# TheCacophonyProject/audio-training

Measured on AMD Instinct MI355X. Metric: clips/sec training (3s@48kHz, wr_resnet) at 1/2/4/8 GPU; mel pipeline GB/s, higher is better.
Workload: dtype bf16

## Files before the change

audio-training_amd/acfe/_lib.py:

```python
from __future__ import annotations

import ctypes as C
import os
from pathlib import Path

LIB_PATH = Path(os.environ.get("ACFE_LIB") or Path(__file__).resolve().parent / "libacfe.so")

P = C.c_void_p
I32 = C.c_int
I64 = C.c_int64
F32 = C.c_float
F64 = C.c_double

SIGNATURES: dict[str, list] = {
    "acfe_version": [],
    "acfe_last_error": [],
    "acfe_crc32c": [P, C.c_size_t, C.c_uint32],
    "acfe_tfr_open": [C.c_char_p, I32, P],
    "acfe_tfr_next": [P, I32, P, P],
    "acfe_tfr_close": [P],
    "acfe_example_audio": [P, C.c_uint64, C.c_char_p, P, I64, P, I32, P],
    "acfe_mel_filterbank": [I32, I32, F64, F64, I32, F64, P],
    "acfe_plan_create": [I32, I32, I32, I32, F64, F64, F64, P, P],
    "acfe_plan_destroy": [P],
# ... 27 lines not shown
    "acfe_conv2d_wgrad_bnbwd_rows": [I32] * 5,
    "acfe_conv2d_wgrad_bnbwd": [P, I32, I32, I32, I32, P, P, I32, P, P, I32, P, P, F32, C.c_uint64, P, P, F32, P, P,
                                P],
    "acfe_conv2d_dropout_keep_supported": [I32] * 6,
    "acfe_conv2d_fwd_dropout_keep": [P, I32, I32, I32, I32, P, I32, I32, I32, P, P, P, F32, C.c_uint64, P, P],
    "acfe_conv2d_fwd_bn_keep": [P, I32, I32, I32, I32, P, I32, I32, I32, P, P, P, F32, C.c_uint64, P, P, I32, P, P,
                                I32, P],
    "acfe_conv2d_wgrad_bnbwd_keep": [P, I32, I32, I32, I32, P, P, I32, P, P, I32, P, F32, C.c_uint64, P, P, P, F32,
                                     P, P, P],
    "acfe_stem_blocks": [I32, I32, I32],
    "acfe_stem_fold_weights": [P, I32, I32, I32, I32, P, P],
    "acfe_stem_fwd": [P, I32, I32, I32, I32, I32, I32, I32, I32, P, P, P, I32, P, P],
    "acfe_stem_dgrad": [P, I32, I32, I32, I32, I32, I32, I32, I32, P, P, I32, P],
    "acfe_stem_wgrad": [P, I32, P, I32, I32, I32, I32, I32, I32, I32, I32, I32, P, F32, P, P],
    "acfe_stem_bwd_bn": [P, P, P, I32, I32, I32, I32, I32, I32, I32, P, P, P, P, I32, P, I32, P, F32, P, P, P],
    "acfe_reduce_blocks": [I64],
    "acfe_bn_stats": [P, I64, I32, I32, P, P],
    "acfe_bn_finalize": [P, I32, I32, I32, F64, P, P, F32, F32, P, P, I32, P, P, P, P, P],
    "acfe_bn_apply": [P, I32, I64, I32, P, P, I32, P, I32, P],
    "acfe_bn_bwd_reduce": [P, I32, P, I32, I64, I32, P, P, P, P, I32, P, P],
    "acfe_bn_bwd_finalize": [P, I32, I32, F64, P, P, P, P, P, P, P],
    "acfe_bn_bwd_finalize_ex": [P, I32, I32, F64, P, P, P, P, P, P, I32, P],
    "acfe_bn_bwd_apply": [P, I32, P, I32, I64, I32, P, P, I32, P, P, P, I32, P],
    "acfe_bn_bwd_apply_dropout": [P, I32, P, I32, I64, I32, P, P, I32, P, F32, C.c_uint64, P, I32, P],
    "acfe_bn_bwd_apply_ex": [P, I32, P, I32, I64, I32, P, P, I32, P, P, F32, C.c_uint64, P, I32, P, P],
    "acfe_conv2d_pool_supported": [I32, I32, I32, I32, I32, I32, I32, I32],
    "acfe_conv2d_fwd_pool": [P, I32, I32, I32, I32, P, I32, I32, I32, P, P, P, F32, C.c_uint64, P, I32, P],
    "acfe_conv2d_dgrad_unpool": [P, P, I32, I32, I32, I32, P, I32, I32, I32, P, I32, P],
    "acfe_conv2d_wgrad_unpool": [P, I32, I32, I32, I32, P, P, I32, I32, I32, P, F32, I32, P, P],
    "acfe_bn_bwd_apply_pool": [P, I32, P, I32, I32, I32, I32, I32, P, P, I32, P, P, I32, P, I32, P, P],
# ... 17 lines not shown
    "acfe_channel_sum": [P, I64, I32, I32, P, P, F32, P],
    "acfe_add": [P, P, I64, I32, P, I32, P],
    "acfe_add_stats": [P, P, I64, I32, I32, P, I32, P, P],
    "acfe_relu_bwd_sum": [P, P, I64, I32, P, I32, P, P],
    "acfe_channel_sum_finalize": [P, I32, I32, F32, P, P],
    "acfe_relu_bwd": [P, P, I64, P, I32, P],
    "acfe_dropout": [P, I64, F32, C.c_uint64, P, I32, P],
    "acfe_cast": [P, I32, I64, P, I32, P],
    "acfe_sigmoid": [P, I64, P, P],
    "acfe_maxpool2d": [P, I32, I32, I32, I32, I32, I32, P, I32, P],
    "acfe_maxpool2d_bwd": [P, P, I32, I32, I32, I32, I32, I32, P, I32, P],
    "acfe_maxpool2d_fused": [P, I32, I32, I32, I32, I32, I32, P, P, F32, C.c_uint64, P, I32, P],
    "acfe_bn_maxpool2d_fused": [P, I32, I32, I32, I32, P, P, I32, I32, I32, P, P, P, I32, P],
    "acfe_maxpool2d_bwd_argmax": [P, P, I32, I32, I32, I32, I32, I32, F32, C.c_uint64, P, I32, P],
    "acfe_maxpool2d_bwd_argmax_bn": [P, P, I32, I32, I32, I32, I32, I32, P, I32, P, P, P, P, P, I32, P, P],
    "acfe_avgpool2d": [P, I32, I32, I32, I32, I32, P, I32, P],
    "acfe_avgpool2d_bwd": [P, I32, I32, I32, I32, I32, P, I32, P],
    "acfe_axis_pool": [P, I32, I64, I32, I32, F32, I32, P, P],
    "acfe_axis_pool_bwd": [P, I32, P, I64, I32, I32, F32, I32, P, P],
    "acfe_dense_fwd": [P, P, P, I32, I32, I32, P, P],
    "acfe_dense_bwd": [P, P, P, I32, I32, I32, P, P, P, P],
    "acfe_loss": [P, P, I32, I32, I32, F32, P, P, P, P],
    "acfe_adam_step": [P, P, P, P, I64, F32, F32, F32, F32, F32, P],
}
_RESTYPES = {"acfe_last_error": C.c_char_p, "acfe_conv2d_wgrad_workspace": I64, "acfe_conv2d_dgrad_workspace": I64, "acfe_crc32c": C.c_uint32,
             "acfe_c1bn_workspace": I64}

PAD_END, PAD_CENTER_CONSTANT, PAD_CENTER_REFLECT = 0, 1, 2
LAYOUT_BTM, LAYOUT_BMT = 0, 1
DTYPE_F32, DTYPE_BF16 = 0, 1
# ... 40 lines not shown
```

audio-training_amd/acfe/ops.py:

```python
from __future__ import annotations

import itertools
import os

import torch

from ._lib import call, lib
from ._torch import dtype_code, ptr, stream

F32, F64 = torch.float32, torch.float64

FUSE = os.environ.get("ACFE_FUSE", "1") != "0"
UNPOOL = os.environ.get("ACFE_UNPOOL", "1") != "0"
PROLOGUE = os.environ.get("ACFE_BN_PROLOGUE", "1") != "0"
PRO_POOL = os.environ.get("ACFE_BN_PROLOGUE_POOL", "1") != "0"
PRO_C1 = os.environ.get("ACFE_BN_PROLOGUE_C1", "0") != "0"
PRO_1W = os.environ.get("ACFE_BN_PROLOGUE_1W", "1") != "0"
FUSE_BN_REDUCE = FUSE and os.environ.get("ACFE_BN_REDUCE_FUSE", "1") != "0"
STEM_BN_FUSE = os.environ.get("ACFE_STEM_BN_FUSE", "1") != "0"
FUSE_BN_BWD = FUSE and os.environ.get("ACFE_BN_BWD_FUSE", "1") != "0"
KEEP_BITS = os.environ.get("ACFE_KEEP_BITS", "1") != "0"
FUSE_SUB = FUSE and os.environ.get("ACFE_SUB_FUSE", "1") != "0"


def same_padding(n: int, k: int, s: int) -> tuple[int, int]:
    out = -(-n // s)
    total = max((out - 1) * s + k - n, 0)
    return out, total // 2


def valid_out(n: int, k: int, s: int) -> int:
    return (n - k) // s + 1


# ... 371 lines not shown
        ctx.save_for_backward(x, w, weff, y, amax, *saved)
        ctx.conf, ctx.gb = conf, (gamma, beta)
        ctx.mark_non_differentiable(pst)
        return yp, pst

    @staticmethod
    def backward(ctx, g, _gs):
        x, w, weff, y, amax, *saved = ctx.saved_tensors
        pt, pl, out_dtype, kh, kw, relu, eps, momentum, want_stats = ctx.conf
        N, H, W, K = y.shape
        _, R, S, rep = w.shape
        dev = y.device
        s = stream()
        scale, shift, mean, invstd = saved
        g = g.contiguous()
        gu = _empty(y.shape, g.dtype, dev)
        rows = N * H * W
        nrows = lib.acfe_reduce_blocks(rows)
        part = _empty((nrows * 2 * K,), F64, dev)
        call("acfe_maxpool2d_bwd_argmax_bn", ptr(amax), ptr(g), N, H, W, K, kh, kw, ptr(gu), dtype_code(g.dtype),
             ptr(y), ptr(scale), ptr(shift), ptr(mean), ptr(invstd), int(relu), ptr(part), s)
        coef, dgamma, dbeta = _bn_bwd_coef(part, nrows, K, rows, saved, True, ctx.gb, dev)
        nb = lib.acfe_stem_blocks(N, H, W)
        dx = _empty(x.shape, x.dtype, dev)
        dw = _empty(w.shape, F32, dev)
        ws = _empty((nb * K * R * S,), F64, dev)
        bp = _empty((nb, 2, K), F64, dev)
        call("acfe_stem_bwd_bn", ptr(gu), ptr(y), ptr(x), N, H, W, R, S, pt, pl, ptr(weff), ptr(scale), ptr(shift),
             ptr(coef), int(relu), ptr(dx), rep, ptr(dw), 0.0, ptr(bp), ptr(ws), s)
        db = None
        if ctx.needs_input_grad[2]:
            db = _empty((K,), F32, dev)
            call("acfe_channel_sum_finalize", ptr(bp), nb, K, 0.0, ptr(db), s)
        return (dx if ctx.needs_input_grad[0] else None), dw, db, dgamma, dbeta, None, None, None


def stem_bn_pool_ok(x, w, b, out_dtype, kh, kw) -> bool:
    K, R, S, _ = w.shape
    return (FUSE and FUSE_BN_REDUCE and STEM_BN_FUSE and torch.is_grad_enabled() and b is not None
            and x.dtype == torch.bfloat16 and out_dtype == torch.bfloat16 and x.dim() == 3 and x.is_contiguous()
            and K == 16 and R == S and R in (3, 5) and (kh, kw) in ((1, 2), (2, 2), (3, 3)))


def stem_bn_max_pool(x, w, b, out_dtype, gamma, beta, mmean, mvar, kh, kw, relu=False, eps=1e-3, momentum=0.99,
# ... 1094 lines not shown
```

audio-training_amd/csrc/conv.hip:

```cpp
#include "conv_common.h"

#if !defined(ACFE_ABLATE) && (defined(ACFE_FB_NOXFORM) || defined(ACFE_FB_NOSUM) || defined(ACFE_FB_NOSTORE) || \
                              defined(ACFE_FB_MID))
#error "ACFE_FB_* ablation switches belong to `make ablate` builds only"
#endif

using namespace acfe;



__device__ __attribute__((aligned(64))) uint4 g_zero_page[4];


template <typename T> struct TT;
template <> struct TT<uint16_t> { static constexpr int GR = 8, BK = 64; };
template <> struct TT<float> { static constexpr int GR = 4, BK = 32; };

__device__ __forceinline__ void mma(f4& acc, const uint4& a, const uint4& b, uint16_t) {
  acc = __builtin_amdgcn_mfma_f32_16x16x32_bf16(__builtin_bit_cast(bf8, a), __builtin_bit_cast(bf8, b), acc,
                                                0, 0, 0);
}
__device__ __forceinline__ void mma(f4& acc, const uint4& a, const uint4& b, float) {
  acc = __builtin_amdgcn_mfma_f32_16x16x4f32(__uint_as_float(a.x), __uint_as_float(b.x), acc, 0, 0, 0);
  acc = __builtin_amdgcn_mfma_f32_16x16x4f32(__uint_as_float(a.y), __uint_as_float(b.y), acc, 0, 0, 0);
// ... 4852 lines not shown
  }
#pragma unroll
  for (int r = 0; r < 4; ++r) {
    red[wid][q * 4 + r][l16] = d0[r];
    red[wid][q * 4 + r][16 + l16] = d1[r];
  }
  __syncthreads();
  for (int i = tid; i < STEM_K * NT; i += 256) {
    const int k = i / NT, t = i - k * NT;
    part[(long long)blockIdx.x * STEM_K * NT + i] =
        ((double)red[0][k][t] + (double)red[1][k][t]) + ((double)red[2][k][t] + (double)red[3][k][t]);
  }
}


template <int R, int S>
__global__ void __launch_bounds__(256) __attribute__((amdgpu_waves_per_eu(3)))
k_stem_bwd_bn(const uint16_t* __restrict__ g, const uint16_t* __restrict__ xb, const uint16_t* __restrict__ xin,
              int N, int H, int W, int pt, int pl, const float* __restrict__ weff, const float* __restrict__ scale,
              const float* __restrict__ shift, const float* __restrict__ coef, int relu, uint16_t* __restrict__ dxin,
              double* __restrict__ wpart, double* __restrict__ bpart, int tiles_h, int tiles_w) {
  constexpr int XH = STEM_TH + R - 1, XW = STEM_TW + S - 1, NT = R * S, NKT = (NT + 1) / 2;
  constexpr int GSZ = XH * XW * STEM_K;
  static_assert(GSZ * 2 >= 4 * STEM_K * 32 * 4, "the wgrad reduction aliases the dY image");
  __shared__ __attribute__((aligned(16))) uint16_t gs[GSZ];
  __shared__ uint16_t xs[XH * XW];
  __shared__ double bred[4][STEM_K];
  __shared__ __attribute__((aligned(16))) float bnc[5][STEM_K];
  const int tid = threadIdx.x, lane = tid & 63, l16 = lane & 15, q = lane >> 4, wid = tid >> 6;
  if (tid < 5 * STEM_K) {
    const int a = tid / STEM_K, k = tid - a * STEM_K;
    bnc[a][k] = a == 0 ? scale[k] : (a == 1 ? shift[k] : coef[(a - 2) * STEM_K + k]);
  }
  uint4 wa[NKT];
  int goff[NKT];
#pragma unroll
  for (int kt = 0; kt < NKT; ++kt) {
    const int t = 2 * kt + (q >> 1), r = t / S, s = t % S;
    float v[8];
#pragma unroll
    for (int j = 0; j < 8; ++j) v[j] = t < NT ? weff[t * STEM_K + (q & 1) * 8 + j] : 0.f;
    wa[kt] = uint4{stem_pack2(v[0], v[1]), stem_pack2(v[2], v[3]), stem_pack2(v[4], v[5]), stem_pack2(v[6], v[7])};
    goff[kt] = t < NT ? ((R - 1 - r) * XW + (S - 1 - s)) * STEM_K + (q & 1) * 8 : -1;
  }
  const int grp = lane >> 4, qq = (lane & 15) >> 2, pp = lane & 3;
  int tof0, tof1;
  {
    const int t0 = l16, t1 = 16 + l16;
    tof0 = t0 < NT ? (t0 / S) * XW + (t0 % S) : -1;
    tof1 = t1 < NT ? (t1 / S) * XW + (t1 % S) : -1;
  }
  const int c8 = (tid & 1) * 8;
  double s1[8];
#pragma unroll
  for (int j = 0; j < 8; ++j) s1[j] = 0.0;
  f4 d0 = f4{0.f, 0.f, 0.f, 0.f}, d1 = d0;
  const uint4 z4 = {0u, 0u, 0u, 0u};
  const long long ntiles = (long long)N * tiles_h * tiles_w;
  for (long long tt = blockIdx.x; tt < ntiles; tt += gridDim.x) {
    const int tw = (int)(tt % tiles_w), th = (int)((tt / tiles_w) % tiles_h);
    const int n = (int)(tt / ((long long)tiles_w * tiles_h));
    const int h0 = th * STEM_TH, w0 = tw * STEM_TW;
    const int gh0 = h0 - (R - 1 - pt), gw0 = w0 - (S - 1 - pl);
    __syncthreads();
    for (int i = tid; i < XH * XW * 2; i += 256) {
      const int pos = i >> 1;
      const int yy = pos / XW, xx = pos - yy * XW;
      const int h = gh0 + yy, w = gw0 + xx;
      u32x4 v = {0u, 0u, 0u, 0u};
      if ((unsigned)h < (unsigned)H && (unsigned)w < (unsigned)W) {
        const long long e = (((long long)n * H + h) * W + w) * STEM_K + c8;
        const u32x4 gv = *reinterpret_cast<const u32x4*>(g + e);
        const u32x4 xv = *reinterpret_cast<const u32x4*>(xb + e);
        float o[8];
#pragma unroll
        for (int j = 0; j < 8; ++j) {
          const unsigned gw = gv[j >> 1], xw = xv[j >> 1];
          const float gf = __uint_as_float((j & 1) ? (gw & 0xffff0000u) : (gw << 16));
          const float xf = __uint_as_float((j & 1) ? (xw & 0xffff0000u) : (xw << 16));
          const float gj = (relu && !(xf * bnc[0][c8 + j] + bnc[1][c8 + j] > 0.f)) ? 0.f : gf;
          o[j] = __builtin_fmaf(bnc[2][c8 + j], gj, __builtin_fmaf(bnc[3][c8 + j], xf, bnc[4][c8 + j]));
        }
        v = u32x4{stem_pack2(o[0], o[1]), stem_pack2(o[2], o[3]), stem_pack2(o[4], o[5]), stem_pack2(o[6], o[7])};
        if ((unsigned)(yy - (R - 1 - pt)) < (unsigned)STEM_TH && (unsigned)(xx - (S - 1 - pl)) < (unsigned)STEM_TW) {
#pragma unroll
          for (int j = 0; j < 8; ++j) {
            const unsigned vw = v[j >> 1];
            s1[j] += (double)__uint_as_float((j & 1) ? (vw & 0xffff0000u) : (vw << 16));
          }
        }
      }
      *reinterpret_cast<u32x4*>(gs + (long long)i * 8) = v;
    }
    for (int i = tid; i < XH * XW; i += 256) {
      const int yy = i / XW, xx = i - yy * XW;
      const int h = h0 - pt + yy, w = w0 - pl + xx;
      xs[i] = ((unsigned)h < (unsigned)H && (unsigned)w < (unsigned)W) ? xin[((long long)n * H + h) * W + w] : 0;
    }
    __syncthreads();
#pragma unroll 2
    for (int blk = 0; blk < 16; ++blk) {
      const int ry = wid * 4 + (blk >> 2), cx = (blk & 3) * 16 + l16;
      const uint16_t* base = gs + (ry * XW + cx) * STEM_K;
      f4 acc = f4{0.f, 0.f, 0.f, 0.f};
#pragma unroll
      for (int kt = 0; kt < NKT; ++kt) {
        const uint4 b = goff[kt] >= 0 ? *reinterpret_cast<const uint4*>(base + goff[kt]) : z4;
        acc = __builtin_amdgcn_mfma_f32_16x16x32_bf16(__builtin_bit_cast(bf8, wa[kt]), __builtin_bit_cast(bf8, b), acc,
                                                      0, 0, 0);
      }
      const int h = h0 + ry, w = w0 + cx;
      if (q == 0 && h < H && w < W) dxin[((long long)n * H + h) * W + w] = f2bf(acc[0]);
    }
    for (int c = 0; c < 8; ++c) {
// ... 5 lines not shown
          (stem_lp)(reinterpret_cast<const __bf16*>(gw + (16 + 4 * grp + qq) * STEM_K + 4 * pp)));
      const bf8 a = bf8{lo[0], lo[1], lo[2], lo[3], hi[0], hi[1], hi[2], hi[3]};
      const uint16_t* src = xs + ry * XW + cx0;
      unsigned b0[8], b1[8];
#pragma unroll
      for (int j = 0; j < 8; ++j) {
        const int px = j < 4 ? 4 * q + j : 16 + 4 * q + (j - 4);
        b0[j] = tof0 >= 0 ? src[px + tof0] : 0u;
        b1[j] = tof1 >= 0 ? src[px + tof1] : 0u;
      }
      const uint4 B0 = uint4{b0[0] | (b0[1] << 16), b0[2] | (b0[3] << 16), b0[4] | (b0[5] << 16), b0[6] | (b0[7] << 16)};
      const uint4 B1 = uint4{b1[0] | (b1[1] << 16), b1[2] | (b1[3] << 16), b1[4] | (b1[5] << 16), b1[6] | (b1[7] << 16)};
      d0 = __builtin_amdgcn_mfma_f32_16x16x32_bf16(a, __builtin_bit_cast(bf8, B0), d0, 0, 0, 0);
      d1 = __builtin_amdgcn_mfma_f32_16x16x32_bf16(a, __builtin_bit_cast(bf8, B1), d1, 0, 0, 0);
    }
  }
#pragma unroll
  for (int j = 0; j < 8; ++j) {
#pragma unroll
    for (int o = 2; o < 64; o <<= 1) s1[j] += __shfl_xor(s1[j], o, 64);
  }
  __syncthreads();
  float(*red)[STEM_K][32] = reinterpret_cast<float(*)[STEM_K][32]>(gs);
#pragma unroll
  for (int r = 0; r < 4; ++r) {
    red[wid][q * 4 + r][l16] = d0[r];
    red[wid][q * 4 + r][16 + l16] = d1[r];
  }
  if (lane < 2) {
#pragma unroll
// ... 103 lines not shown
      hipLaunchKernelGGL((k_stem_wgrad_mfma<3, 3>), dim3(grid), dim3(256), 0, strm(stream), (const uint16_t*)x,
                         (const uint16_t*)dy, N, H, W, pad_top, pad_left, workspace, th, tw);
  } else if (x_dtype == ACFE_DTYPE_BF16 && dy_dtype == ACFE_DTYPE_BF16) SW(uint16_t, uint16_t);
  else if (x_dtype == ACFE_DTYPE_BF16) SW(uint16_t, float);
  else if (dy_dtype == ACFE_DTYPE_BF16) SW(float, uint16_t);
  else SW(float, float);
#undef SW
  int rc = launch_rc("acfe_stem_wgrad");
  if (rc) return rc;
  const int n = STEM_K * R * S;
  if (rep > 256) return ACFE_E_INVAL;
  hipLaunchKernelGGL(k_stem_wgrad_reduce, dim3(n), dim3(256), 0, strm(stream), workspace, grid, n, rep, beta, dw);
  return launch_rc("acfe_stem_wgrad(reduce)");
}

ACFE_API int acfe_stem_bwd_bn(const void* g, const void* xb, const void* xin, int N, int H, int W, int R, int S,
                              int pad_top, int pad_left, const float* weff, const float* scale, const float* shift,
                              const float* coef, int relu, void* dxin, int rep, float* dw, float beta,
                              double* bias_part, double* workspace, void* stream) {
  if (!g || !xb || !xin || !weff || !scale || !shift || !coef || !dw || !bias_part || !workspace || N <= 0 ||
      H <= 0 || W <= 0 || R != S || (R != 5 && R != 3) || rep <= 0 || rep > 256 || ((uintptr_t)g & 15) ||
      ((uintptr_t)xb & 15))
    return ACFE_E_INVAL;
  const int th = (H + STEM_TH - 1) / STEM_TH, tw = (W + STEM_TW - 1) / STEM_TW;
  const int nb = acfe_stem_blocks(N, H, W), grid = stem_bwd_grid(N, H, W);
  if (grid < nb) {
    const hipError_t e =
        hipMemsetAsync(bias_part + (size_t)grid * 2 * STEM_K, 0, sizeof(double) * 2 * STEM_K * (nb - grid), strm(stream));
    if (e != hipSuccess) return hip_rc(e, "acfe_stem_bwd_bn");
  }
  uint16_t* dxo = (uint16_t*)dxin;
  if (!dxo) return ACFE_E_INVAL;
#define SB(RR)                                                                                                \
  hipLaunchKernelGGL((k_stem_bwd_bn<RR, RR>), dim3(grid), dim3(256), 0, strm(stream), (const uint16_t*)g,        \
                     (const uint16_t*)xb, (const uint16_t*)xin, N, H, W, pad_top, pad_left, weff, scale, shift, coef, \
                     relu, dxo, workspace, bias_part, th, tw)
  if (R == 5) SB(5); else SB(3);
#undef SB
  int rc = launch_rc("acfe_stem_bwd_bn");
  if (rc) return rc;
  const int n = STEM_K * R * S;
  hipLaunchKernelGGL(k_stem_wgrad_reduce, dim3(n), dim3(256), 0, strm(stream), workspace, grid, n, rep, beta, dw);
  return launch_rc("acfe_stem_bwd_bn(reduce)");
}
```

audio-training_amd/csrc/nn.hip:

```cpp
#include "common.h"

using namespace acfe;

template <typename T> __device__ __forceinline__ float ld(const T* p, long long i);
template <> __device__ __forceinline__ float ld<uint16_t>(const uint16_t* p, long long i) { return bf2f(p[i]); }
template <> __device__ __forceinline__ float ld<float>(const float* p, long long i) { return p[i]; }
template <typename T> __device__ __forceinline__ void st(T* p, long long i, float v);
template <> __device__ __forceinline__ void st<uint16_t>(uint16_t* p, long long i, float v) { p[i] = f2bf(v); }
template <> __device__ __forceinline__ void st<float>(float* p, long long i, float v) { p[i] = v; }

#define DISPATCH1(dt, T, ...)                                   \
  do {                                                          \
    if ((dt) == ACFE_DTYPE_BF16) { typedef uint16_t T; __VA_ARGS__; } \
    else { typedef float T; __VA_ARGS__; }                      \
  } while (0)

static int grid_for(long long n, int per = 256, int cap = 8192) {
  long long g = (n + per - 1) / per;
  if (g < 1) g = 1;
  return (int)(g < cap ? g : cap);
}

static int red_blocks(long long rows) {
  long long b = (rows + 255) / 256;
// ... 1053 lines not shown
        st8(dx + (((size_t)n * H + p * KH + a) * W + q * KW + b) * C + cv * 8, o);
      }
    const float z[8] = {0, 0, 0, 0, 0, 0, 0, 0};
    if (q == Q - 1)
      for (int a = 0; a < KH; ++a)
        for (int w = Q * KW; w < W; ++w) st8(dx + (((size_t)n * H + p * KH + a) * W + w) * C + cv * 8, z);
    if (p == P - 1)
      for (int h = P * KH; h < H; ++h) {
        for (int w = q * KW; w < q * KW + KW; ++w) st8(dx + (((size_t)n * H + h) * W + w) * C + cv * 8, z);
        if (q == Q - 1)
          for (int w = Q * KW; w < W; ++w) st8(dx + (((size_t)n * H + h) * W + w) * C + cv * 8, z);
      }
  }
}

template <typename T, int KH, int KW>
__global__ void __launch_bounds__(256) k_maxpool_bwd8i_bn(const uint8_t* __restrict__ amax, const T* __restrict__ dy,
                                                          int N, int H, int W, int C, int P, int Q,
                                                          T* __restrict__ dx, const T* __restrict__ x,
                                                          const float* __restrict__ scale,
                                                          const float* __restrict__ shift,
                                                          const float* __restrict__ mean,
                                                          const float* __restrict__ invstd, int relu,
                                                          double* __restrict__ part) {
  extern __shared__ double red[];
  for (int i = threadIdx.x; i < 2 * C; i += 256) red[i] = 0.0;
  __syncthreads();
  constexpr int JU = 2;
  const int CV = C >> 3, lcv = __builtin_ctz(CV), RV = Q * CV;
  const int cv = threadIdx.x & (CV - 1);
  float sc[8], sh[8], mu[8], is[8], a[8], b[8];
// ... 33 lines not shown
#pragma unroll
        for (int k = 0; k < 4; ++k) am[k] = (pk[u].x >> (8 * k)) & 0xff, am[4 + k] = (pk[u].y >> (8 * k)) & 0xff;
#pragma unroll
        for (int aa = 0; aa < KH; ++aa)
#pragma unroll
          for (int bb = 0; bb < KW; ++bb) {
            const float* xw = xv[u][aa * KW + bb];
            float o[8];
#pragma unroll
            for (int k = 0; k < 8; ++k) {
              o[k] = am[k] == aa * KW + bb ? g[u][k] : 0.f;
              const float gk = (relu && !(xw[k] * sc[k] + sh[k] > 0.f)) ? 0.f : o[k];
              a[k] += gk;
              b[k] += gk * ((xw[k] - mu[k]) * is[k]);
            }
            st8(dx + (fin + ((size_t)aa * W + q * KW + bb) * CV + cv) * 8, o);
          }
        if (q == Q - 1)
          for (int aa = 0; aa < KH; ++aa)
            for (int w = Q * KW; w < W; ++w) st8(dx + (fin + ((size_t)aa * W + w) * CV + cv) * 8, z);
        if (p == P - 1)
          for (int h = P * KH; h < H; ++h) {
            const size_t hr = ((size_t)n * H + h) * W;
            for (int w = q * KW; w < q * KW + KW; ++w) st8(dx + ((hr + w) * CV + cv) * 8, z);
            if (q == Q - 1)
              for (int w = Q * KW; w < W; ++w) st8(dx + ((hr + w) * CV + cv) * 8, z);
          }
      }
    }
    if (++cnt == 16) {
#pragma unroll
      for (int j = 0; j < 8; ++j) da[j] += a[j], db[j] += b[j], a[j] = b[j] = 0.f;
// ... 76 lines not shown
      kw <= 0 || H < kh || W < kw || !stats8_ok(C))
    return ACFE_E_INVAL;
  const int P = H / kh, Q = W / kw;
  if (!vec_ok((long long)N * H * W * C, C, dy, dx, x) || ((uintptr_t)argmax & 7) || (long long)N * P >= (1ll << 31))
    return ACFE_E_INVAL;
  const int grid = red_blocks((long long)N * H * W);
#define MPBB(A, B)                                                                                             \
  if (kh == A && kw == B) {                                                                                    \
    DISPATCH1(dtype, T, hipLaunchKernelGGL((k_maxpool_bwd8i_bn<T, A, B>), dim3(grid), dim3(256),               \
                                           2 * C * sizeof(double), strm(stream), argmax, (const T*)dy, N, H, W, C, \
                                           P, Q, (T*)dx, (const T*)x, scale, shift, mean, invstd, relu, part));   \
    return launch_rc("acfe_maxpool2d_bwd_argmax_bn");                                                          \
  }
  MAXPOOL_SHAPES(MPBB)
#undef MPBB
  return ACFE_E_INVAL;
}

template <typename T>
__global__ void __launch_bounds__(256) k_add8s(const T* __restrict__ a, const T* __restrict__ b, unsigned nvec,
                                               int C, int relu, T* __restrict__ z, double* __restrict__ part) {
  extern __shared__ double red[];
  for (int i = threadIdx.x; i < 2 * C; i += 256) red[i] = 0.0;
  __syncthreads();
  const int CV = C >> 3;
  double sa[8], sb[8];
#pragma unroll
  for (int j = 0; j < 8; ++j) sa[j] = sb[j] = 0.0;
  const unsigned v0 = blockIdx.x * 256 + threadIdx.x;
  for (unsigned v = v0; v < nvec; v += gridDim.x * 256) {
// ... 452 lines not shown
```

include/acfe.h:

```cpp
#ifndef ACFE_H
#define ACFE_H

#include <stdint.h>
#include <stddef.h>

#ifdef __cplusplus
extern "C" {
#endif

#define ACFE_OK 0
#define ACFE_E_INVAL (-1000)
#define ACFE_E_NOMEM (-1001)

#define ACFE_PAD_END 0
#define ACFE_PAD_CENTER_CONSTANT 1
#define ACFE_PAD_CENTER_REFLECT 2

#define ACFE_LAYOUT_BTM 0
#define ACFE_LAYOUT_BMT 1

#define ACFE_DTYPE_F32 0
#define ACFE_DTYPE_BF16 1

typedef struct acfe_plan_s* acfe_plan_t;
// ... 96 lines not shown

int acfe_stem_blocks(int N, int H, int W);
int acfe_stem_fold_weights(const float* w_krsc, int K, int R, int S, int C, float* weff, void* stream);
int acfe_stem_fwd(const void* x, int x_dtype, int N, int H, int W, int R, int S, int pad_top, int pad_left,
                  const float* weff, const float* bias, void* y, int y_dtype, double* stats_partial,
                  void* stream);
int acfe_stem_dgrad(const void* dy, int dy_dtype, int N, int H, int W, int R, int S, int pad_top,
                    int pad_left, const float* weff, void* dx, int dx_dtype, void* stream);
int acfe_stem_wgrad(const void* x, int x_dtype, const void* dy, int dy_dtype, int N, int H, int W, int R,
                    int S, int pad_top, int pad_left, int rep, float* dw, float beta, double* workspace,
                    void* stream);
int acfe_stem_bwd_bn(const void* g, const void* xb, const void* xin, int N, int H, int W, int R, int S,
                     int pad_top, int pad_left, const float* weff, const float* scale, const float* shift,
                     const float* coef, int relu, void* dxin, int rep, float* dw, float beta,
                     double* bias_part, double* workspace, void* stream);

int acfe_reduce_blocks(long long rows);
int acfe_bn_stats(const void* x, long long rows, int C, int dtype, double* partial, void* stream);
int acfe_bn_finalize(const double* partial, int nrows, int ld, int C, double count, const float* gamma,
                     const float* beta, float eps, float momentum, float* moving_mean, float* moving_var,
                     int training, float* scale, float* shift, float* mean, float* invstd, void* stream);
int acfe_bn_apply(const void* x, int x_dtype, long long rows, int C, const float* scale, const float* shift,
                  int relu, void* y, int y_dtype, void* stream);
int acfe_bn_bwd_reduce(const void* dy, int dy_dtype, const void* x, int x_dtype, long long rows, int C,
                       const float* scale, const float* shift, const float* mean, const float* invstd,
                       int relu, double* partial, void* stream);
int acfe_bn_bwd_finalize(const double* partial, int nrows, int C, double count, const float* scale,
                         const float* mean, const float* invstd, float* dgamma, float* dbeta, float* coef,
                         void* stream);
int acfe_bn_bwd_finalize_ex(const double* partial, int nrows, int C, double count, const float* scale,
// ... 86 lines not shown

int acfe_maxpool2d(const void* x, int N, int H, int W, int C, int kh, int kw, void* y, int dtype,
                   void* stream);
int acfe_maxpool2d_bwd(const void* x, const void* dy, int N, int H, int W, int C, int kh, int kw, void* dx,
                       int dtype, void* stream);
int acfe_maxpool2d_fused(const void* x, int N, int H, int W, int C, int kh, int kw, void* y, uint8_t* argmax,
                         float drop_rate, unsigned long long seed, double* partial, int dtype, void* stream);
int acfe_bn_maxpool2d_fused(const void* x, int N, int H, int W, int C, const float* scale, const float* shift,
                            int relu, int kh, int kw, void* y, uint8_t* argmax, double* stats_part, int dtype,
                            void* stream);
int acfe_maxpool2d_bwd_argmax(const uint8_t* argmax, const void* dy, int N, int H, int W, int C, int kh, int kw,
                              float drop_rate, unsigned long long seed, void* dx, int dtype, void* stream);
int acfe_maxpool2d_bwd_argmax_bn(const uint8_t* argmax, const void* dy, int N, int H, int W, int C, int kh, int kw,
                                 void* dx, int dtype, const void* x, const float* scale, const float* shift,
                                 const float* mean, const float* invstd, int relu, double* part, void* stream);
int acfe_avgpool2d(const void* x, int N, int H, int W, int C, int k, void* y, int dtype, void* stream);
int acfe_avgpool2d_bwd(const void* dy, int N, int H, int W, int C, int k, void* dx, int dtype, void* stream);
int acfe_axis_pool(const void* x, int x_dtype, long long outer, int L, int inner, float sharpness, int mode,
                   float* y, void* stream);
int acfe_axis_pool_bwd(const void* x, int x_dtype, const float* dy, long long outer, int L, int inner,
                       float sharpness, int mode, void* dx, void* stream);

int acfe_dense_fwd(const float* x, const float* w, const float* bias, int B, int I, int O, float* z,
                   void* stream);
int acfe_dense_bwd(const float* x, const float* w, const float* dz, int B, int I, int O, float* dx, float* dw,
                   float* db, void* stream);
int acfe_loss(const float* z, const float* y, int B, int L, int mode, float grad_scale, float* loss, float* dz,
              float* workspace, void* stream);

int acfe_adam_step(float* params, const float* grads, float* m, float* v, long long n, float grad_scale,
// ... 7 lines not shown
```

Measured before the change: 11850.

## Fuse maxpool unpooling into stem BN backward to skip the unpooled gradient buffer

The stem backward no longer writes a full-resolution unpooled gradient. The maxpool backward now only computes the BN reduction sums. The stem BN-backward kernel reads the pooled gradient and argmax directly and unpools on the fly while filling its shared-memory tile. The kernel also restructures tile loading into column pairs with clamped loads, and moves the packed weights into LDS to cut register pressure. This removes a full-size bf16 write and re-read, in exchange for more index arithmetic and extra template variants.

```diff
diff --git a/audio-training_amd/acfe/_lib.py b/audio-training_amd/acfe/_lib.py
--- a/audio-training_amd/acfe/_lib.py
+++ b/audio-training_amd/acfe/_lib.py
@@ -65,6 +65,8 @@
     "acfe_stem_dgrad": [P, I32, I32, I32, I32, I32, I32, I32, I32, P, P, I32, P],
     "acfe_stem_wgrad": [P, I32, P, I32, I32, I32, I32, I32, I32, I32, I32, I32, P, F32, P, P],
     "acfe_stem_bwd_bn": [P, P, P, I32, I32, I32, I32, I32, I32, I32, P, P, P, P, I32, P, I32, P, F32, P, P, P],
+    "acfe_stem_bwd_bn_unpool": [P, P, I32, I32, P, P, I32, I32, I32, I32, I32, I32, I32, P, P, P, P, I32, P, I32, P,
+                                F32, P, P, P],
     "acfe_reduce_blocks": [I64],
     "acfe_bn_stats": [P, I64, I32, I32, P, P],
     "acfe_bn_finalize": [P, I32, I32, I32, F64, P, P, F32, F32, P, P, I32, P, P, P, P, P],
@@ -112,6 +114,7 @@
     "acfe_bn_maxpool2d_fused": [P, I32, I32, I32, I32, P, P, I32, I32, I32, P, P, P, I32, P],
     "acfe_maxpool2d_bwd_argmax": [P, P, I32, I32, I32, I32, I32, I32, F32, C.c_uint64, P, I32, P],
     "acfe_maxpool2d_bwd_argmax_bn": [P, P, I32, I32, I32, I32, I32, I32, P, I32, P, P, P, P, P, I32, P, P],
+    "acfe_maxpool2d_bwd_argmax_bn_sums": [P, P, I32, I32, I32, I32, I32, I32, I32, P, P, P, P, P, I32, P, P],
     "acfe_avgpool2d": [P, I32, I32, I32, I32, I32, P, I32, P],
     "acfe_avgpool2d_bwd": [P, I32, I32, I32, I32, I32, P, I32, P],
     "acfe_axis_pool": [P, I32, I64, I32, I32, F32, I32, P, P],
diff --git a/audio-training_amd/acfe/ops.py b/audio-training_amd/acfe/ops.py
--- a/audio-training_amd/acfe/ops.py
+++ b/audio-training_amd/acfe/ops.py
@@ -18,6 +18,7 @@
 PRO_1W = os.environ.get("ACFE_BN_PROLOGUE_1W", "1") != "0"
 FUSE_BN_REDUCE = FUSE and os.environ.get("ACFE_BN_REDUCE_FUSE", "1") != "0"
 STEM_BN_FUSE = os.environ.get("ACFE_STEM_BN_FUSE", "1") != "0"
+STEM_UNPOOL = os.environ.get("ACFE_STEM_UNPOOL", "1") != "0"
 FUSE_BN_BWD = FUSE and os.environ.get("ACFE_BN_BWD_FUSE", "1") != "0"
 KEEP_BITS = os.environ.get("ACFE_KEEP_BITS", "1") != "0"
 FUSE_SUB = FUSE and os.environ.get("ACFE_SUB_FUSE", "1") != "0"
@@ -419,20 +420,30 @@
         s = stream()
         scale, shift, mean, invstd = saved
         g = g.contiguous()
-        gu = _empty(y.shape, g.dtype, dev)
         rows = N * H * W
         nrows = lib.acfe_reduce_blocks(rows)
         part = _empty((nrows * 2 * K,), F64, dev)
-        call("acfe_maxpool2d_bwd_argmax_bn", ptr(amax), ptr(g), N, H, W, K, kh, kw, ptr(gu), dtype_code(g.dtype),
-             ptr(y), ptr(scale), ptr(shift), ptr(mean), ptr(invstd), int(relu), ptr(part), s)
+        unpool = STEM_UNPOOL and (kh, kw) in ((1, 2), (2, 2))
+        if unpool:
+            call("acfe_maxpool2d_bwd_argmax_bn_sums", ptr(amax), ptr(g), N, H, W, K, kh, kw, dtype_code(g.dtype),
+                 ptr(y), ptr(scale), ptr(shift), ptr(mean), ptr(invstd), int(relu), ptr(part), s)
+        else:
+            gu = _empty(y.shape, g.dtype, dev)
+            call("acfe_maxpool2d_bwd_argmax_bn", ptr(amax), ptr(g), N, H, W, K, kh, kw, ptr(gu), dtype_code(g.dtype),
+                 ptr(y), ptr(scale), ptr(shift), ptr(mean), ptr(invstd), int(relu), ptr(part), s)
         coef, dgamma, dbeta = _bn_bwd_coef(part, nrows, K, rows, saved, True, ctx.gb, dev)
         nb = lib.acfe_stem_blocks(N, H, W)
         dx = _empty(x.shape, x.dtype, dev)
         dw = _empty(w.shape, F32, dev)
         ws = _empty((nb * K * R * S,), F64, dev)
         bp = _empty((nb, 2, K), F64, dev)
-        call("acfe_stem_bwd_bn", ptr(gu), ptr(y), ptr(x), N, H, W, R, S, pt, pl, ptr(weff), ptr(scale), ptr(shift),
-             ptr(coef), int(relu), ptr(dx), rep, ptr(dw), 0.0, ptr(bp), ptr(ws), s)
+        if unpool:
+            call("acfe_stem_bwd_bn_unpool", ptr(g), ptr(amax), kh, kw, ptr(y), ptr(x), N, H, W, R, S, pt, pl,
+                 ptr(weff), ptr(scale), ptr(shift), ptr(coef), int(relu), ptr(dx), rep, ptr(dw), 0.0, ptr(bp),
+                 ptr(ws), s)
+        else:
+            call("acfe_stem_bwd_bn", ptr(gu), ptr(y), ptr(x), N, H, W, R, S, pt, pl, ptr(weff), ptr(scale),
+                 ptr(shift), ptr(coef), int(relu), ptr(dx), rep, ptr(dw), 0.0, ptr(bp), ptr(ws), s)
         db = None
         if ctx.needs_input_grad[2]:
             db = _empty((K,), F32, dev)
diff --git a/audio-training_amd/csrc/conv.hip b/audio-training_amd/csrc/conv.hip
--- a/audio-training_amd/csrc/conv.hip
+++ b/audio-training_amd/csrc/conv.hip
@@ -4890,14 +4890,21 @@
 }
 
 
-template <int R, int S>
+struct StemPf {
+  u32x4 g0, g1, x0, x1;
+};
+
+template <int R, int S, int KH>
 __global__ void __launch_bounds__(256) __attribute__((amdgpu_waves_per_eu(3)))
-k_stem_bwd_bn(const uint16_t* __restrict__ g, const uint16_t* __restrict__ xb, const uint16_t* __restrict__ xin,
-              int N, int H, int W, int pt, int pl, const float* __restrict__ weff, const float* __restrict__ scale,
-              const float* __restrict__ shift, const float* __restrict__ coef, int relu, uint16_t* __restrict__ dxin,
-              double* __restrict__ wpart, double* __restrict__ bpart, int tiles_h, int tiles_w) {
+k_stem_bwd_bn(const uint16_t* __restrict__ g, const uint8_t* __restrict__ amax, int P, int Q,
+              const uint16_t* __restrict__ xb, const uint16_t* __restrict__ xin, int N, int H, int W, int pt, int pl,
+              const float* __restrict__ weff, const float* __restrict__ scale, const float* __restrict__ shift,
+              const float* __restrict__ coef, int relu, uint16_t* __restrict__ dxin, double* __restrict__ wpart,
+              double* __restrict__ bpart, int tiles_h, int tiles_w) {
   constexpr int XH = STEM_TH + R - 1, XW = STEM_TW + S - 1, NT = R * S, NKT = (NT + 1) / 2;
   constexpr int GSZ = XH * XW * STEM_K;
+  constexpr int PW = XW / 2 + 1, NPU = XH * PW, NR = (NPU * 2 + 255) / 256, NXR = (XH * XW + 255) / 256;
+  static_assert(XW % 2 == 0 && STEM_TW % 2 == 0, "column pairs");
   static_assert(GSZ * 2 >= 4 * STEM_K * 32 * 4, "the wgrad reduction aliases the dY image");
   __shared__ __attribute__((aligned(16))) uint16_t gs[GSZ];
   __shared__ uint16_t xs[XH * XW];
@@ -4908,7 +4915,7 @@
     const int a = tid / STEM_K, k = tid - a * STEM_K;
     bnc[a][k] = a == 0 ? scale[k] : (a == 1 ? shift[k] : coef[(a - 2) * STEM_K + k]);
   }
-  uint4 wa[NKT];
+  __shared__ uint4 wlds[NKT][4];
   int goff[NKT];
 #pragma unroll
   for (int kt = 0; kt < NKT; ++kt) {
@@ -4916,7 +4923,8 @@
     float v[8];
 #pragma unroll
     for (int j = 0; j < 8; ++j) v[j] = t < NT ? weff[t * STEM_K + (q & 1) * 8 + j] : 0.f;
-    wa[kt] = uint4{stem_pack2(v[0], v[1]), stem_pack2(v[2], v[3]), stem_pack2(v[4], v[5]), stem_pack2(v[6], v[7])};
+    if (wid == 0 && l16 == 0)
+      wlds[kt][q] = uint4{stem_pack2(v[0], v[1]), stem_pack2(v[2], v[3]), stem_pack2(v[4], v[5]), stem_pack2(v[6], v[7])};
     goff[kt] = t < NT ? ((R - 1 - r) * XW + (S - 1 - s)) * STEM_K + (q & 1) * 8 : -1;
   }
   const int grp = lane >> 4, qq = (lane & 15) >> 2, pp = lane & 3;
@@ -4927,38 +4935,72 @@
     tof1 = t1 < NT ? (t1 / S) * XW + (t1 % S) : -1;
   }
   const int c8 = (tid & 1) * 8;
+  const int dh = R - 1 - pt, dw = S - 1 - pl, ao = dw & 1;
   double s1[8];
 #pragma unroll
   for (int j = 0; j < 8; ++j) s1[j] = 0.0;
   f4 d0 = f4{0.f, 0.f, 0.f, 0.f}, d1 = d0;
   const uint4 z4 = {0u, 0u, 0u, 0u};
   const long long ntiles = (long long)N * tiles_h * tiles_w;
-  for (long long tt = blockIdx.x; tt < ntiles; tt += gridDim.x) {
-    const int tw = (int)(tt % tiles_w), th = (int)((tt / tiles_w) % tiles_h);
-    const int n = (int)(tt / ((long long)tiles_w * tiles_h));
-    const int h0 = th * STEM_TH, w0 = tw * STEM_TW;
-    const int gh0 = h0 - (R - 1 - pt), gw0 = w0 - (S - 1 - pl);
-    __syncthreads();
-    for (int i = tid; i < XH * XW * 2; i += 256) {
-      const int pos = i >> 1;
-      const int yy = pos / XW, xx = pos - yy * XW;
-      const int h = gh0 + yy, w = gw0 + xx;
+
+  auto issue = [&](int n, int h0, int w0, int r) -> StemPf {
+    int pu = (tid >> 1) + 128 * r;
+    if (pu >= NPU) pu = NPU - 1;
+    const int yy = pu / PW, pc = pu - yy * PW;
+    const int h = h0 - dh + yy, w = w0 - dw + 2 * pc - ao;
+    const int hc = min(max(h, 0), H - 1), wa0 = min(max(w, 0), W - 1), wa1 = min(max(w + 1, 0), W - 1);
+    const long long img = (long long)n * H * W * STEM_K;
+    const int e0 = (hc * W + wa0) * STEM_K + c8, e1 = (hc * W + wa1) * STEM_K + c8;
+    StemPf p;
+    p.x0 = *reinterpret_cast<const u32x4*>(xb + img + e0);
+    p.x1 = *reinterpret_cast<const u32x4*>(xb + img + e1);
+    if constexpr (KH == 0) {
+      p.g0 = *reinterpret_cast<const u32x4*>(g + img + e0);
+      p.g1 = *reinterpret_cast<const u32x4*>(g + img + e1);
+    } else {
+      const int hp = min(max(h, 0), P * KH - 1) / KH, qc = min(max(w >> 1, 0), Q - 1);
+      const long long e = (((long long)n * P + hp) * Q + qc) * STEM_K + c8;
+      p.g0 = *reinterpret_cast<const u32x4*>(g + e);
+      const uint2 a = *reinterpret_cast<const uint2*>(amax + e);
+      p.g1 = u32x4{a.x, a.y, 0u, 0u};
+    }
+    return p;
+  };
+  auto consume = [&](const StemPf& p, int h0, int w0, int r) {
+    const int pu = (tid >> 1) + 128 * r;
+    if ((NPU * 2) % 256 != 0 && r == NR - 1 && pu >= NPU) return;
+    const int yy = pu / PW, pc = pu - yy * PW;
+    const int xx0 = 2 * pc - ao;
+    const int h = h0 - dh + yy, w = w0 - dw + xx0;
+    const bool hv = (unsigned)h < (unsigned)H;
+    const bool wv = KH > 0 && (unsigned)h < (unsigned)(P * KH) && (unsigned)w < (unsigned)(2 * Q);
+    const unsigned tap0 = KH == 2 ? (unsigned)(h & 1) * 2u : 0u;
+#pragma unroll
+    for (int jj = 0; jj < 2; ++jj) {
+      const int xx = xx0 + jj;
+      if ((unsigned)xx >= (unsigned)XW) continue;
       u32x4 v = {0u, 0u, 0u, 0u};
-      if ((unsigned)h < (unsigned)H && (unsigned)w < (unsigned)W) {
-        const long long e = (((long long)n * H + h) * W + w) * STEM_K + c8;
-        const u32x4 gv = *reinterpret_cast<const u32x4*>(g + e);
-        const u32x4 xv = *reinterpret_cast<const u32x4*>(xb + e);
+      if (hv && (unsigned)(w + jj) < (unsigned)W) {
+        const u32x4 xv = jj ? p.x1 : p.x0;
         float o[8];
 #pragma unroll
         for (int j = 0; j < 8; ++j) {
-          const unsigned gw = gv[j >> 1], xw = xv[j >> 1];
-          const float gf = __uint_as_float((j & 1) ? (gw & 0xffff0000u) : (gw << 16));
+          const unsigned xw = xv[j >> 1];
           const float xf = __uint_as_float((j & 1) ? (xw & 0xffff0000u) : (xw << 16));
+          float gf;
+          if constexpr (KH == 0) {
+            const unsigned gw = (jj ? p.g1 : p.g0)[j >> 1];
+            gf = __uint_as_float((j & 1) ? (gw & 0xffff0000u) : (gw << 16));
+          } else {
+            const unsigned gw = p.g0[j >> 1];
+            const unsigned am = (p.g1[j >> 2] >> (8 * (j & 3))) & 0xffu;
+            gf = (wv && am == tap0 + jj) ? __uint_as_float((j & 1) ? (gw & 0xffff0000u) : (gw << 16)) : 0.f;
+          }
           const float gj = (relu && !(xf * bnc[0][c8 + j] + bnc[1][c8 + j] > 0.f)) ? 0.f : gf;
           o[j] = __builtin_fmaf(bnc[2][c8 + j], gj, __builtin_fmaf(bnc[3][c8 + j], xf, bnc[4][c8 + j]));
         }
         v = u32x4{stem_pack2(o[0], o[1]), stem_pack2(o[2], o[3]), stem_pack2(o[4], o[5]), stem_pack2(o[6], o[7])};
-        if ((unsigned)(yy - (R - 1 - pt)) < (unsigned)STEM_TH && (unsigned)(xx - (S - 1 - pl)) < (unsigned)STEM_TW) {
+        if ((unsigned)(yy - dh) < (unsigned)STEM_TH && (unsigned)(xx - dw) < (unsigned)STEM_TW) {
 #pragma unroll
           for (int j = 0; j < 8; ++j) {
             const unsigned vw = v[j >> 1];
@@ -4966,14 +5008,43 @@
           }
         }
       }
-      *reinterpret_cast<u32x4*>(gs + (long long)i * 8) = v;
-    }
-    for (int i = tid; i < XH * XW; i += 256) {
-      const int yy = i / XW, xx = i - yy * XW;
-      const int h = h0 - pt + yy, w = w0 - pl + xx;
-      xs[i] = ((unsigned)h < (unsigned)H && (unsigned)w < (unsigned)W) ? xin[((long long)n * H + h) * W + w] : 0;
-    }
+      *reinterpret_cast<u32x4*>(gs + (yy * XW + xx) * STEM_K + c8) = v;
+    }
+  };
+  auto tile_at = [&](long long t, int& n, int& h0, int& w0) {
+    const int tw = (int)(t % tiles_w), th = (int)((t / tiles_w) % tiles_h);
+    n = (int)(t / ((long long)tiles_w * tiles_h));
+    h0 = th * STEM_TH, w0 = tw * STEM_TW;
+  };
+
+  long long tt = blockIdx.x;
+  int n, h0, w0;
+  tile_at(tt, n, h0, w0);
+  for (;;) {
     __syncthreads();
+#pragma unroll 1
+    for (int r = 0; r < NR; ++r) consume(issue(n, h0, w0, r), h0, w0, r);
+    {
+      uint16_t xr[NXR];
+#pragma unroll
+      for (int k = 0; k < NXR; ++k) {
+        const int i = min(tid + 256 * k, XH * XW - 1);
+        const int yy = i / XW, xx = i - yy * XW;
+        const int hc = min(max(h0 - pt + yy, 0), H - 1), wc = min(max(w0 - pl + xx, 0), W - 1);
+        xr[k] = xin[((long long)n * H + hc) * W + wc];
+      }
+#pragma unroll
+      for (int k = 0; k < NXR; ++k) {
+        const int i = tid + 256 * k;
+        const int yy = i / XW, xx = i - yy * XW;
+        const int h = h0 - pt + yy, w = w0 - pl + xx;
+        if (i < XH * XW) xs[i] = ((unsigned)h < (unsigned)H && (unsigned)w < (unsigned)W) ? xr[k] : (uint16_t)0;
+      }
+    }
+    __syncthreads();
+    uint4 wa[NKT];
+#pragma unroll
+    for (int kt = 0; kt < NKT; ++kt) wa[kt] = wlds[kt][q];
 #pragma unroll 2
     for (int blk = 0; blk < 16; ++blk) {
       const int ry = wid * 4 + (blk >> 2), cx = (blk & 3) * 16 + l16;
@@ -5009,6 +5080,9 @@
       d0 = __builtin_amdgcn_mfma_f32_16x16x32_bf16(a, __builtin_bit_cast(bf8, B0), d0, 0, 0, 0);
       d1 = __builtin_amdgcn_mfma_f32_16x16x32_bf16(a, __builtin_bit_cast(bf8, B1), d1, 0, 0, 0);
     }
+    tt += gridDim.x;
+    if (tt >= ntiles) break;
+    tile_at(tt, n, h0, w0);
   }
 #pragma unroll
   for (int j = 0; j < 8; ++j) {
@@ -5142,32 +5216,56 @@
   return launch_rc("acfe_stem_wgrad(reduce)");
 }
 
-ACFE_API int acfe_stem_bwd_bn(const void* g, const void* xb, const void* xin, int N, int H, int W, int R, int S,
-                              int pad_top, int pad_left, const float* weff, const float* scale, const float* shift,
-                              const float* coef, int relu, void* dxin, int rep, float* dw, float beta,
-                              double* bias_part, double* workspace, void* stream) {
-  if (!g || !xb || !xin || !weff || !scale || !shift || !coef || !dw || !bias_part || !workspace || N <= 0 ||
+static int stem_bwd_bn_impl(const void* g, const uint8_t* amax, int kh, int kw, const void* xb, const void* xin,
+                            int N, int H, int W, int R, int S, int pad_top, int pad_left, const float* weff,
+                            const float* scale, const float* shift, const float* coef, int relu, void* dxin, int rep,
+                            float* dw, float beta, double* bias_part, double* workspace, void* stream,
+                            const char* name) {
+  if (!g || !xb || !xin || !weff || !scale || !shift || !coef || !dxin || !dw || !bias_part || !workspace || N <= 0 ||
       H <= 0 || W <= 0 || R != S || (R != 5 && R != 3) || rep <= 0 || rep > 256 || ((uintptr_t)g & 15) ||
-      ((uintptr_t)xb & 15))
+      ((uintptr_t)xb & 15) || pad_top < 0 || pad_top >= R || pad_left < 0 || pad_left >= S ||
+      (long long)H * W * STEM_K >= (1ll << 31))
     return ACFE_E_INVAL;
+  const int P = kh ? H / kh : 0, Q = kh ? W / kw : 0;
+  if (kh && (!amax || ((uintptr_t)amax & 7) || kw != 2 || (kh != 1 && kh != 2) || P <= 0 || Q <= 0)) return ACFE_E_INVAL;
   const int th = (H + STEM_TH - 1) / STEM_TH, tw = (W + STEM_TW - 1) / STEM_TW;
   const int nb = acfe_stem_blocks(N, H, W), grid = stem_bwd_grid(N, H, W);
   if (grid < nb) {
     const hipError_t e =
         hipMemsetAsync(bias_part + (size_t)grid * 2 * STEM_K, 0, sizeof(double) * 2 * STEM_K * (nb - grid), strm(stream));
-    if (e != hipSuccess) return hip_rc(e, "acfe_stem_bwd_bn");
-  }
-  uint16_t* dxo = (uint16_t*)dxin;
-  if (!dxo) return ACFE_E_INVAL;
-#define SB(RR)                                                                                                \
-  hipLaunchKernelGGL((k_stem_bwd_bn<RR, RR>), dim3(grid), dim3(256), 0, strm(stream), (const uint16_t*)g,        \
-                     (const uint16_t*)xb, (const uint16_t*)xin, N, H, W, pad_top, pad_left, weff, scale, shift, coef, \
-                     relu, dxo, workspace, bias_part, th, tw)
-  if (R == 5) SB(5); else SB(3);
+    if (e != hipSuccess) return hip_rc(e, name);
+  }
+#define SB(RR, KH)                                                                                                 \
+  hipLaunchKernelGGL((k_stem_bwd_bn<RR, RR, KH>), dim3(grid), dim3(256), 0, strm(stream), (const uint16_t*)g, amax, P, \
+                     Q, (const uint16_t*)xb, (const uint16_t*)xin, N, H, W, pad_top, pad_left, weff, scale, shift,   \
+                     coef, relu, (uint16_t*)dxin, workspace, bias_part, th, tw)
+  if (R == 5) {
+    if (kh == 0) SB(5, 0); else if (kh == 1) SB(5, 1); else SB(5, 2);
+  } else {
+    if (kh == 0) SB(3, 0); else if (kh == 1) SB(3, 1); else SB(3, 2);
+  }
 #undef SB
-  int rc = launch_rc("acfe_stem_bwd_bn");
+  int rc = launch_rc(name);
   if (rc) return rc;
   const int n = STEM_K * R * S;
   hipLaunchKernelGGL(k_stem_wgrad_reduce, dim3(n), dim3(256), 0, strm(stream), workspace, grid, n, rep, beta, dw);
-  return launch_rc("acfe_stem_bwd_bn(reduce)");
-}
+  return launch_rc(name);
+}
+
+ACFE_API int acfe_stem_bwd_bn(const void* g, const void* xb, const void* xin, int N, int H, int W, int R, int S,
+                              int pad_top, int pad_left, const float* weff, const float* scale, const float* shift,
+                              const float* coef, int relu, void* dxin, int rep, float* dw, float beta,
+                              double* bias_part, double* workspace, void* stream) {
+  return stem_bwd_bn_impl(g, nullptr, 0, 0, xb, xin, N, H, W, R, S, pad_top, pad_left, weff, scale, shift, coef, relu,
+                          dxin, rep, dw, beta, bias_part, workspace, stream, "acfe_stem_bwd_bn");
+}
+
+ACFE_API int acfe_stem_bwd_bn_unpool(const void* gp, const uint8_t* argmax, int kh, int kw, const void* xb,
+                                     const void* xin, int N, int H, int W, int R, int S, int pad_top, int pad_left,
+                                     const float* weff, const float* scale, const float* shift, const float* coef,
+                                     int relu, void* dxin, int rep, float* dw, float beta, double* bias_part,
+                                     double* workspace, void* stream) {
+  if (!argmax || kw != 2 || (kh != 1 && kh != 2) || H < kh || W < kw) return ACFE_E_INVAL;
+  return stem_bwd_bn_impl(gp, argmax, kh, kw, xb, xin, N, H, W, R, S, pad_top, pad_left, weff, scale, shift, coef, relu,
+                          dxin, rep, dw, beta, bias_part, workspace, stream, "acfe_stem_bwd_bn_unpool");
+}
diff --git a/audio-training_amd/csrc/nn.hip b/audio-training_amd/csrc/nn.hip
--- a/audio-training_amd/csrc/nn.hip
+++ b/audio-training_amd/csrc/nn.hip
@@ -1091,7 +1091,7 @@
   }
 }
 
-template <typename T, int KH, int KW>
+template <typename T, int KH, int KW, bool WR = true>
 __global__ void __launch_bounds__(256) k_maxpool_bwd8i_bn(const uint8_t* __restrict__ amax, const T* __restrict__ dy,
                                                           int N, int H, int W, int C, int P, int Q,
                                                           T* __restrict__ dx, const T* __restrict__ x,
@@ -1155,8 +1155,9 @@
               a[k] += gk;
               b[k] += gk * ((xw[k] - mu[k]) * is[k]);
             }
-            st8(dx + (fin + ((size_t)aa * W + q * KW + bb) * CV + cv) * 8, o);
+            if (WR) st8(dx + (fin + ((size_t)aa * W + q * KW + bb) * CV + cv) * 8, o);
           }
+        if (!WR) continue;
         if (q == Q - 1)
           for (int aa = 0; aa < KH; ++aa)
             for (int w = Q * KW; w < W; ++w) st8(dx + (fin + ((size_t)aa * W + w) * CV + cv) * 8, z);
@@ -1263,6 +1264,29 @@
   }
   MAXPOOL_SHAPES(MPBB)
 #undef MPBB
+  return ACFE_E_INVAL;
+}
+
+ACFE_API int acfe_maxpool2d_bwd_argmax_bn_sums(const uint8_t* argmax, const void* dy, int N, int H, int W, int C,
+                                               int kh, int kw, int dtype, const void* x, const float* scale,
+                                               const float* shift, const float* mean, const float* invstd, int relu,
+                                               double* part, void* stream) {
+  if (!argmax || !dy || !x || !scale || !shift || !mean || !invstd || !part || N <= 0 || kh <= 0 || kw <= 0 ||
+      H < kh || W < kw || !stats8_ok(C))
+    return ACFE_E_INVAL;
+  const int P = H / kh, Q = W / kw;
+  if (!vec_ok((long long)N * H * W * C, C, dy, x) || ((uintptr_t)argmax & 7) || (long long)N * P >= (1ll << 31))
+    return ACFE_E_INVAL;
+  const int grid = red_blocks((long long)N * H * W);
+#define MPBS(A, B)                                                                                             \
+  if (kh == A && kw == B) {                                                                                    \
+    DISPATCH1(dtype, T, hipLaunchKernelGGL((k_maxpool_bwd8i_bn<T, A, B, false>), dim3(grid), dim3(256),        \
+                                           2 * C * sizeof(double), strm(stream), argmax, (const T*)dy, N, H, W, C, \
+                                           P, Q, (T*)nullptr, (const T*)x, scale, shift, mean, invstd, relu, part)); \
+    return launch_rc("acfe_maxpool2d_bwd_argmax_bn_sums");                                                     \
+  }
+  MAXPOOL_SHAPES(MPBS)
+#undef MPBS
   return ACFE_E_INVAL;
 }
 
diff --git a/include/acfe.h b/include/acfe.h
--- a/include/acfe.h
+++ b/include/acfe.h
@@ -134,6 +134,10 @@
                      int pad_top, int pad_left, const float* weff, const float* scale, const float* shift,
                      const float* coef, int relu, void* dxin, int rep, float* dw, float beta,
                      double* bias_part, double* workspace, void* stream);
+int acfe_stem_bwd_bn_unpool(const void* gp, const uint8_t* argmax, int kh, int kw, const void* xb, const void* xin,
+                            int N, int H, int W, int R, int S, int pad_top, int pad_left, const float* weff,
+                            const float* scale, const float* shift, const float* coef, int relu, void* dxin,
+                            int rep, float* dw, float beta, double* bias_part, double* workspace, void* stream);
 
 int acfe_reduce_blocks(long long rows);
 int acfe_bn_stats(const void* x, long long rows, int C, int dtype, double* partial, void* stream);
@@ -250,6 +254,9 @@
 int acfe_maxpool2d_bwd_argmax_bn(const uint8_t* argmax, const void* dy, int N, int H, int W, int C, int kh, int kw,
                                  void* dx, int dtype, const void* x, const float* scale, const float* shift,
                                  const float* mean, const float* invstd, int relu, double* part, void* stream);
+int acfe_maxpool2d_bwd_argmax_bn_sums(const uint8_t* argmax, const void* dy, int N, int H, int W, int C, int kh,
+                                      int kw, int dtype, const void* x, const float* scale, const float* shift,
+                                      const float* mean, const float* invstd, int relu, double* part, void* stream);
 int acfe_avgpool2d(const void* x, int N, int H, int W, int C, int k, void* y, int dtype, void* stream);
 int acfe_avgpool2d_bwd(const void* dy, int N, int H, int W, int C, int k, void* dx, int dtype, void* stream);
 int acfe_axis_pool(const void* x, int x_dtype, long long outer, int L, int inner, float sharpness, int mode,
```

Result: no change. 11810, median of 2 (-0.3%).
